# sean-lo/OptimalMatrixCompletion.jl

Hardware: AMD Instinct MI355X
Metric: B&B node-relaxations/sec, 100x100 k=1 (higher is better)
Workload: dtype f64

## Files before the change

optimalmatrixcompletion.jl_amd/csrc/omc_api.cpp:

```cpp
#include <hip/hip_runtime.h>
#include <stdint.h>
#include <limits.h>
#include <stdio.h>
#include <stdlib.h>
#include <string.h>
#include <math.h>
#include <chrono>
#include <string>
#include <vector>
#include <algorithm>
#include <atomic>
#include <thread>
#include <mutex>

#include "omc.h"
#include "omc_device.h"
#include "omc_altmin.h"
#include "omc_shor.h"
#include "omc_shor_relax.h"
#include <unordered_map>
#include <dlfcn.h>
#include <execinfo.h>
#include <signal.h>
#include <unistd.h>
#include <rccl/rccl.h>

#include "omc_host.h"

thread_local std::string g_err;

static void knob_set(Tuning& t, const Knob& kb, const char* value) {
  if (kb.flag) t.*kb.flag = value != nullptr;
  else t.*kb.num = value ? atoi(value) : Tuning{}.*kb.num;
}
static void omc_segv_trace(int sig) {
  void* fr[64];
  const int nf = backtrace(fr, 64);
  const char msg[] = "libomc_hip: fatal signal, native frames:\n";
  (void)!write(2, msg, sizeof(msg) - 1);
  backtrace_symbols_fd(fr, nf, 2);
  signal(sig, SIG_DFL);
  raise(sig);
}
static void tuning_from_env(Tuning& t) {
  for (const Knob& kb : OMC_KNOBS) knob_set(t, kb, getenv(kb.name));
}


extern "C" {

const char* omc_last_error(void) { return g_err.c_str(); }
int omc_version(void) { return OMC_VERSION; }
int omc_device_count(void) {
  int c = 0;
  if (hipGetDeviceCount(&c) != hipSuccess) return 0;
  return c;
}

void omc_relax_params_default(omc_relax_params* p) {
  p->eps_gap = 1e-6; p->eps_feas = 1e-7; p->max_iters = 3000; p->check_every = 25;
  p->rho_scale = 1.0; p->rho_f_ratio = 0.1; p->relax = 1.6; p->time_limit = 3600.0;
  p->reference_quirk_q1 = 1; p->breakpoints = OMC_SMALLEST_1_EIGVEC; p->stall_checks = 8;
  p->bump_max = 2; p->bump_ratio = 4.0; p->bump_factor = 4.0; p->bump_after = 100; p->bump_window = 4; p->slots = 0;
  p->accel = 0; p->aa_mem = 10; p->aa_every = 10; p->aa_start = 50; p->aa_reg = 1e-10; p->aa_safeguard = 1.0; p->first_wins = 0;
  p->early_stop_after = 400; p->early_stop_factor = 1.5;
}

static int upload(DevBuf& b, const void* src, size_t bytes, hipStream_t s) {
  int rc = b.ensure(bytes ? bytes : 8);
  if (rc) return rc;
  if (bytes) HIPCHK(hipMemcpyAsync(b.p, src, bytes, hipMemcpyHostToDevice, s));
  return 0;
}

static int build_colprox_lists(omc_instance* h, int block_min, bool pair_on) {
  if (h->lists_valid && h->lists_block_min == block_min && h->lists_pair == pair_on) return 0;
  const int m = h->m, lds_c = cp_block_lds_cmax(), max_c = cp_block_cmax();
  std::vector<int> solo, wide, blk, slab;
  std::vector<uint8_t> isb(m, 0);
  h->cpb_cl = h->cpb_cs = h->crest_max = h->nrest = 0;
  for (int j0 = 0; j0 < m; j0 += 2) {
    const int j1 = j0 + 1;
    const int c0 = h->col_ptr[j0 + 1] - h->col_ptr[j0], c1 = (j1 < m) ? h->col_ptr[j1 + 1] - h->col_ptr[j1] : 0;
    const bool paired = j1 < m && c0 <= 32 && c1 <= 32;
    for (int j = j0; j <= j1 && j < m; ++j) {
      const int c = (j == j0) ? c0 : c1;
      if (c == 0) continue;
      if (!(paired && pair_on) && c >= block_min && c <= max_c) {
        isb[j] = 1;
        if (c <= lds_c) { blk.push_back(j); h->cpb_cl = std::max(h->cpb_cl, c); } else { slab.push_back(j); h->cpb_cs = std::max(h->cpb_cs, c); }
        continue;
      }
      ++h->nrest; h->crest_max = std::max(h->crest_max, c);
      if (paired) continue;
      if (c <= 64) wide.push_back(j); else solo.push_back(j);
    }
  }
  h->nsolo = (int)solo.size(); h->nwide = (int)wide.size(); h->nblock = (int)blk.size(); h->nslab = (int)slab.size();
  int rc = 0;
  if (h->nsolo && (rc = upload(h->dsolo, solo.data(), sizeof(int) * solo.size(), h->stream))) return rc;
  if (h->nwide && (rc = upload(h->dwide, wide.data(), sizeof(int) * wide.size(), h->stream))) return rc;
  if (h->nblock && (rc = upload(h->dblock, blk.data(), sizeof(int) * blk.size(), h->stream))) return rc;
  if (h->nslab && (rc = upload(h->dslab, slab.data(), sizeof(int) * slab.size(), h->stream))) return rc;
  if ((rc = upload(h->disblock, isb.data(), (size_t)m, h->stream))) return rc;
  HIPCHK(hipStreamSynchronize(h->stream));
  h->lists_valid = true; h->lists_block_min = block_min; h->lists_pair = pair_on;
  return 0;
}

int omc_instance_create(int n, int m, int k, const double* A, const uint8_t* mask, double gamma, int device,
                        omc_instance** out) {
  if (!out) return fail(OMC_ERR_ARGUMENT, "out is NULL");
  *out = nullptr;
  if (!A || !mask) return fail(OMC_ERR_ARGUMENT, "A / mask is NULL");
  if (n <= 0 || m <= 0) return fail(OMC_ERR_DIMENSION, "Dimension mismatch: A must have size (n, m) (OMC.jl:240-246)");
  if (!(n <= m)) return fail(OMC_ERR_DIMENSION, "Input matrix A must have size (n, m) with n <= m (OMC.jl:249-254)");
  if (k < 1 || k > n) return fail(OMC_ERR_ARGUMENT, "rank k must satisfy 1 <= k <= n");
  if (k > 8) return fail(OMC_ERR_UNSUPPORTED, "k > 8 is not supported by this build");
  if (!(gamma > 0.0)) return fail(OMC_ERR_ARGUMENT, "gamma must be positive");
  int ndev = 0;
  if (hipGetDeviceCount(&ndev) != hipSuccess || ndev <= 0)
    return fail(OMC_ERR_NO_DEVICE, "no HIP device visible: the HIP path is the product, there is no CPU fallback");
  if (device < 0 || device >= ndev) return fail(OMC_ERR_ARGUMENT, "device index out of range");
  HIPCHK(hipSetDevice(device));
  omc_instance* h = new omc_instance();
  tuning_from_env(h->tun);
  if (h->tun.segv_trace) { signal(SIGSEGV, omc_segv_trace); signal(SIGABRT, omc_segv_trace); }
  struct Guard { omc_instance*& p; ~Guard() { if (p) omc_instance_destroy(p); } } guard{h};
  h->n = n; h->m = m; h->k = k; h->gamma = gamma; h->device = device;
  { int khz = 0; if (hipDeviceGetAttribute(&khz, hipDeviceAttributeWallClockRate, device) == hipSuccess && khz > 0) h->wall_khz = khz; else (void)hipGetLastError(); }
  h->A.assign(A, A + (size_t)n * m);
  h->mask.resize((size_t)n * m);
  for (size_t e = 0; e < (size_t)n * m; ++e) h->mask[e] = mask[e] ? 1 : 0;
  h->col_ptr.assign(m + 1, 0);
  for (int j = 0; j < m; ++j) {
    int c = 0;
    for (int i = 0; i < n; ++i)
      if (h->mask[(size_t)j * n + i]) { h->col_idx.push_back(i); h->col_val.push_back(A[(size_t)j * n + i]); ++c; }
    h->col_ptr[j + 1] = h->col_ptr[j] + c;
    h->cmax = std::max(h->cmax, c);
  }
  h->nnz = h->col_ptr[m];
  h->sumA2 = 0;
  for (double v : h->col_val) h->sumA2 += v * v;
  h->Ncnt.assign((size_t)n * n, 0.0);
  for (int j = 0; j < m; ++j)
    for (int p = h->col_ptr[j]; p < h->col_ptr[j + 1]; ++p)
      for (int q = h->col_ptr[j]; q < h->col_ptr[j + 1]; ++q)
        h->Ncnt[(size_t)h->col_idx[q] * n + h->col_idx[p]] += 1.0;
  h->row_ptr.assign(n + 1, 0);
  for (int i = 0; i < n; ++i) {
    int c = 0;
    for (int j = 0; j < m; ++j)
      if (h->mask[(size_t)j * n + i]) { h->row_idx.push_back(j); h->row_val.push_back(A[(size_t)j * n + i]); ++c; }
    h->row_ptr[i + 1] = h->row_ptr[i] + c;
  }
  HIPCHK(hipStreamCreate(&h->stream));
  int rc = 0;
  if ((rc = upload(h->drow_ptr, h->row_ptr.data(), sizeof(int) * (n + 1), h->stream))) return rc;
  if ((rc = upload(h->drow_idx, h->row_idx.data(), sizeof(int) * h->nnz_rows(), h->stream))) return rc;
  if ((rc = upload(h->drow_val, h->row_val.data(), sizeof(double) * h->nnz_rows(), h->stream))) return rc;
  if ((rc = upload(h->dA, h->A.data(), sizeof(double) * n * m, h->stream))) return rc;
  if ((rc = upload(h->dmask, h->mask.data(), (size_t)n * m, h->stream))) return rc;
  if ((rc = upload(h->dcol_ptr, h->col_ptr.data(), sizeof(int) * (m + 1), h->stream))) return rc;
  if ((rc = build_colprox_lists(h, h->tun.colprox_block_min, !h->tun.no_colprox_pair))) return rc;
  if ((rc = upload(h->dcol_idx, h->col_idx.data(), sizeof(int) * h->nnz, h->stream))) return rc;
  if ((rc = upload(h->dcol_val, h->col_val.data(), sizeof(double) * h->nnz, h->stream))) return rc;
  if ((rc = upload(h->dNcnt, h->Ncnt.data(), sizeof(double) * n * n, h->stream))) return rc;
  HIPCHK(hipStreamSynchronize(h->stream));
  int lrc = omc_set_max_lds();
  if (lrc) return fail(lrc, "hipFuncSetAttribute(MaxDynamicSharedMemorySize) failed");
  { int arc = omc_altmin_set_lds(); if (arc) return fail(5000 + arc, "hipFuncSetAttribute(MaxDynamicSharedMemorySize) failed for the altmin kernel"); }
  omc_relax_params_default(&h->params);
  *out = h;
  h = nullptr;
  return 0;
}

int omc_instance_create_bits(int n, int m, int k, const double* A, const uint64_t* chunks, double gamma, int device,
                             omc_instance** out) {
  if (!chunks) return fail(OMC_ERR_ARGUMENT, "chunks is NULL");
  if (n <= 0 || m <= 0) return fail(OMC_ERR_DIMENSION, "Dimension mismatch (OMC.jl:240-246)");
  std::vector<uint8_t> mask((size_t)n * m);
  for (size_t e = 0; e < (size_t)n * m; ++e) mask[e] = (uint8_t)((chunks[e >> 6] >> (e & 63)) & 1ull);
  return omc_instance_create(n, m, k, A, mask.data(), gamma, device, out);
}

void omc_instance_destroy(omc_instance* h) {
  if (!h) return;
  if (h->worker.joinable()) h->worker.join();
  (void)hipSetDevice(h->device);
  (void)omc_comm_destroy(h);
  for (hipStream_t q : {h->stream, h->gs[0], h->gs[1], h->gs[2], h->append_stream, h->fetch_stream}) if (q) (void)hipStreamDestroy(q);
  for (int q = 0; q < 2; ++q) for (hipEvent_t e : h->ev_pool[q]) (void)hipEventDestroy(e);
  for (hipEvent_t e : h->ev_up) if (e) (void)hipEventDestroy(e);
  if (h->ev_gram) (void)hipEventDestroy(h->ev_gram);
  for (int q = 0; q < 5; ++q) for (hipEvent_t e : {h->gev[q], h->gevc[q]}) if (e) (void)hipEventDestroy(e);
  if (h->ev_main) (void)hipEventDestroy(h->ev_main);
// ... 225 lines not shown
  w.bump_max = P.bump_max; w.bump_ratio = P.bump_ratio; w.bump_factor = P.bump_factor; w.bump_after = P.bump_after;
  w.bump_gap = P.bump_window * std::max(1, P.check_every);
  w.accel = P.accel ? 1 : 0; w.aa_mem = std::max(2, std::min(P.aa_mem, AA_MAXMEM)); w.aa_every = std::max(1, P.aa_every);
  w.aa_start = std::max(2, P.aa_start); w.aa_reg = P.aa_reg; w.aa_safeguard = P.aa_safeguard;
  {
    std::vector<double> hr((size_t)B + extra_nodes, w.rho);
    if (h->rho_scale_per_node.size() == (size_t)B)
      for (int b = 0; b < B; ++b) hr[b] = w.rho / P.rho_scale * h->rho_scale_per_node[b];
    h->rho_scale_per_node.clear();
    int r0 = upload(h->brhon, hr.data(), sizeof(double) * hr.size(), h->stream); if (r0) return r0;
    HIPCHK(hipStreamSynchronize(h->stream));
    w.rho_node = h->brhon.as<double>();
    r0 = h->brho.ensure(sizeof(double) * (size_t)S); if (r0) return r0;
    w.rho_b = h->brho.as<double>();
  }
  w.relax = P.relax; w.eps_gap = P.eps_gap; w.eps_feas = P.eps_feas;
  w.check_every = std::max(1, P.check_every); w.early_stop_after = P.early_stop_after; w.early_stop_factor = (P.first_wins ? 0.0 : P.early_stop_factor);
  {
    int r0 = h->bgap.ensure(sizeof(double) * 2 * (size_t)S); if (r0) return r0;
    r0 = h->bvotes.ensure(sizeof(int) * (size_t)S); if (r0) return r0;
    r0 = h->bslotlist.ensure(sizeof(int) * (size_t)S); if (r0) return r0;
    w.gap_prev = h->bgap.as<double>(); w.gap_rate = h->bgap.as<double>() + S; w.slow_votes = h->bvotes.as<int>();
    w.slot_list = nullptr;
  }
  std::vector<double> wY((size_t)n * n);
  for (size_t e = 0; e < (size_t)n * n; ++e) wY[e] = shor ? 3.0 : P.rho_f_ratio * h->Ncnt[e] + 2.0;
  int rc_ = 0;
  if ((rc_ = upload(h->dwY, wY.data(), sizeof(double) * n * n, h->stream))) return rc_;
  w.col_ptr = h->dcol_ptr.as<int>(); w.col_idx = h->dcol_idx.as<int>(); w.col_val = h->dcol_val.as<double>();
  const int cp_force = h->cp_force;
  h->cp_force = 0;
  {
    const bool pair_on = !h->tun.no_colprox_pair && cp_force != 2;
    if ((rc_ = build_colprox_lists(h, cp_force == 1 ? INT_MAX : cp_force == 2 ? 1 : h->tun.colprox_block_min, pair_on))) return rc_;
    w.cp_pair = pair_on ? 1 : 0;
  }
  w.cp_nblock = h->nblock; w.cp_block = h->nblock ? h->dblock.as<int>() : nullptr;
  w.cp_nslab = h->nslab; w.cp_slab = h->nslab ? h->dslab.as<int>() : nullptr;
  w.cp_isblock = (h->nblock + h->nslab) ? h->disblock.as<unsigned char>() : nullptr; w.cp_nrest = h->nrest; w.cp_nfact = nullptr;
  w.cone_512 = h->tun.cone_512 ? 1 : 0; w.cp_series = CP_SERIES; w.cp_maxpass = CP_MAXPASS; w.cp_xcd = h->tun.colprox_no_xcd ? 0 : 1;
  w.cp_nsolo = h->nsolo; w.cp_solo = h->nsolo ? h->dsolo.as<int>() : nullptr;
  w.cp_nwide = h->nwide; w.cp_wide = h->nwide ? h->dwide.as<int>() : nullptr;
  w.Ncnt = h->dNcnt.as<double>(); w.wY1 = h->dwY.as<double>();
  w.row_ptr = h->drow_ptr.as<int>(); w.row_idx = h->drow_idx.as<int>();
#define ENS(buf, bytes) do { int r_ = (buf).ensure(bytes); if (r_) return r_; } while (0)
  const size_t sB = (size_t)S;
  const size_t sN = (size_t)B + (size_t)extra_nodes;
  ENS(h->bY, sB * n * n * 8); ENS(h->bYp, sB * n * n * 8); ENS(h->bU, sB * n * k * 8);
  ENS(h->bD1, sB * n * n * 8); ENS(h->bD3, sB * n * n * 8); ENS(h->bW1, sB * n * n * 8); ENS(h->bE3, sB * n * n * 8);
  ENS(h->bdS, sB * rmax * rmax * 8);
  ENS(h->bsm, sB * ((size_t)4 * rmax * k + 3 * k * k) * 8);
  ENS(h->balpha, sB * h->nnz * 8); ENS(h->balphaX, sB * h->nnz * 8); ENS(h->bsval, sB * m * 8);
  ENS(h->bMchk, sB * n * n * 8); ENS(h->bchk, sB * n * k * 8 + (32 + 8 * sB) * 8);
  ENS(h->bG, sB * Rmax * Rmax * 8); ENS(h->blam, sB * Rmax * 8);
  ENS(h->bscal, sB * 16 * 8); ENS(h->bbx, sB * n * 8); ENS(h->bint, sB * 10 * sizeof(int));
  w.np16 = (n + 15) & ~15;
  ENS(h->bMbuf, sB * w.np16 * w.np16 * 8); ENS(h->bVrow, sB * w.np16 * w.np16 * 8);
  ENS(h->blamD, sB * m * n * 8);
  HIPCHK(hipMemsetAsync(h->blamD.p, 0, sB * m * n * 8, h->stream));
  w.lamD = h->blamD.as<double>();
  w.lamDX = nullptr;
  if (n > 144 || shor) {
    ENS(h->blamDX, sB * m * n * 8);
    HIPCHK(hipMemsetAsync(h->blamDX.p, 0, sB * m * n * 8, h->stream));
    w.lamDX = h->blamDX.as<double>();
  }
  w.Mbuf = h->bMbuf.as<double>(); w.Vrow = h->bVrow.as<double>();
  {
    ENS(h->bXs, sB * w.np16 * 16 * 8); ENS(h->bsubS, sB * (17 + 256) * 8); ENS(h->bsubI, sB * 15 * sizeof(int));
    HIPCHK(hipMemsetAsync(h->bXs.p, 0, sB * w.np16 * 16 * 8, h->stream));
    HIPCHK(hipMemsetAsync(h->bsubS.p, 0, sB * (17 + 256) * 8, h->stream));
    HIPCHK(hipMemsetAsync(h->bsubI.p, 0, sB * 15 * sizeof(int), h->stream));
    w.Xs = h->bXs.as<double>(); w.sub_theta = h->bsubS.as<double>(); w.trM = h->bsubS.as<double>() + sB * 16;
    w.sub_on = h->bsubI.as<int>(); w.cone_done = h->bsubI.as<int>() + sB; w.sub_stat = h->bsubI.as<int>() + 2 * sB; w.sub_wait = h->bsubI.as<int>() + 10 * sB; w.sub_nfail = h->bsubI.as<int>() + 11 * sB;
    w.V3 = h->bsubS.as<double>() + sB * 17; w.v3valid = h->bsubI.as<int>() + 12 * sB;
// ... 1839 lines not shown
```

optimalmatrixcompletion.jl_amd/csrc/omc_colprox.hip:

```cpp
#include <hip/hip_runtime.h>
#include <type_traits>
#include <stdint.h>
#include "omc_device.h"
#include "omc_wave.h"

template <int Q>
__device__ __forceinline__ double half_bcast(double v) {
  int lo = __double2loint(v), hi = __double2hiint(v);
  lo = __builtin_amdgcn_update_dpp(0, lo, 0x150 + (Q & 15), 0xF, 0xF, false);
  hi = __builtin_amdgcn_update_dpp(0, hi, 0x150 + (Q & 15), 0xF, 0xF, false);
  auto a = __builtin_amdgcn_permlane16_swap(lo, lo, false, false);
  auto c = __builtin_amdgcn_permlane16_swap(hi, hi, false, false);
  return (Q < 16) ? __hiloint2double(c[0], a[0]) : __hiloint2double(c[1], a[1]);
}
__device__ __forceinline__ double half_sum(double v) {
  v = group_sum_dpp<16>(v);
  const int lo = __double2loint(v), hi = __double2hiint(v);
  auto a = __builtin_amdgcn_permlane16_swap(lo, lo, false, false);
  auto c = __builtin_amdgcn_permlane16_swap(hi, hi, false, false);
  return __hiloint2double(c[0], a[0]) + __hiloint2double(c[1], a[1]);
}
#define CPP_LDS_DOUBLES (64 + 64 + 32)

template <int LPC>
__device__ __forceinline__ double lanes_sum(double v) { if constexpr (LPC == 32) return half_sum(v); else return wave_sum(v); }
#define RQ(q) (((q) < 32) ? R0[(q) & 31] : R1[((NC > 32) ? (q) : 0) & 31])
typedef double dbl2_lds __attribute__((ext_vector_type(2), may_alias));
template <int LPC>
__device__ __forceinline__ void colprox_sweep(const OmcWS& w, const int b, const int lane, const int j, const int off, const int c, const int cmax,
                                              double* st, double* vo_s, int* sidx) {
  constexpr int NC = LPC;
  const int h = (LPC == 32) ? (lane >> 5) : 0, l = lane & (LPC - 1), hb = h * LPC;
  const bool act = l < c;
  const int n = w.n;
  const double gm = w.gamma;
  const double* Y = w.Y + (size_t)b * n * n;
  const double* Yp = w.Yp + (size_t)b * n * n;
  const double* Yx = w.Yx ? w.Yx + (size_t)b * n * n : nullptr;
  double* alpha = w.alpha + (size_t)b * w.nnz + off;
  const double a_reg = act ? w.col_val[off + l] : 0.0;
  const int my = act ? w.col_idx[off + l] : 0;
  const double vo_r = act ? alpha[l] : 0.0;
  sidx[lane] = my; vo_s[lane] = vo_r;
  const double rho_f = w.rho_b[b] * w.rho_f_ratio;
  const double coef = gm / (2.0 * rho_f), cp = gm * gm / (2.0 * rho_f);
  double R0[32], R1[(NC > 32) ? 32 : 1], sc;
  const dbl2_lds* st2 = (const dbl2_lds*)st;
  auto gather = [&](double shift) __attribute__((always_inline)) {
#pragma unroll
    for (int qb = 0; qb < NC; qb += 8) {
      if (qb < cmax) {
        double y1[8], y2[8], vq[8];
#pragma unroll
        for (int u = 0; u < 8; ++u) {
          const int iq = sidx[hb + qb + u];
          vq[u] = vo_s[hb + qb + u];
          const size_t a = (l > qb + u) ? (size_t)iq * n + my : (size_t)my * n + iq;
          y1[u] = Yx ? Yx[a] : Y[a]; y2[u] = Yx ? 0.0 : Yp[a];
// ... 59 lines not shown
    st[lane] = v;
    double a0 = 0.0, a1 = 0.0, a2 = 0.0, a3 = 0.0;
#pragma unroll
    for (int qb = 0; qb < NC; qb += 4) {
      if (qb < cm) {
        if constexpr (LPC == 32) {
          const dbl2_lds s01 = st2[(hb + qb) >> 1], s23 = st2[((hb + qb) >> 1) + 1];
          a0 = fma(RQ(qb), s01.x, a0); a1 = fma(RQ(qb + 1), s01.y, a1);
          a2 = fma(RQ(qb + 2), s23.x, a2); a3 = fma(RQ(qb + 3), s23.y, a3);
        } else {
          a0 = fma(RQ(qb), st[hb + qb], a0); a1 = fma(RQ(qb + 1), st[hb + qb + 1], a1);
          a2 = fma(RQ(qb + 2), st[hb + qb + 2], a2); a3 = fma(RQ(qb + 3), st[hb + qb + 3], a3);
        }
      }
    }
    return -sc * ((a0 + a1) + (a2 + a3));
  };
  const double sprev = (j < w.m) ? w.sval[(size_t)b * w.m + j] : 0.0;
  double s = (sprev > 0.0) ? sprev : 0.0;
  double lo = 0.0, hi = -1.0;
  bool lo_valid = false, fin = (c == 0);
  double yout = 0.0;
  const double ser_lim = (w.cp_series >= 6) ? 5e-3 : 1e-5;
  int npass = 0; double dr_first = -1.0; int why = 0;
  for (int it = 0; it <= 60; ++it) {
    if (!__any(!fin)) break;
    const bool last = (it >= w.cp_maxpass);
    gather(cp * s);
    const bool ok_ = invert();
    if (!fin) ++npass;
    double v[6] = {0.0, 0.0, 0.0, 0.0, 0.0, 0.0};
    double rhs = a_reg, yy = 0.0, yz = 0.0, zz = 0.0;
    bool want_ser = false; double dstep = 0.0;
    int K = 2;
    for (int sv = 0; sv < K; ++sv) {
      const double x = apply(rhs);
      rhs = x;
#pragma unroll
      for (int q = 0; q < 6; ++q) v[q] = (sv == q) ? x : v[q];
      if (sv == 0 && last) { if (!fin) { yout = x; fin = true; } break; }
      if (sv == 1) {
        yy = lanes_sum<LPC>(v[0] * v[0]); yz = lanes_sum<LPC>(v[0] * v[1]); zz = lanes_sum<LPC>(v[1] * v[1]);
        bool big = false;
        if (!fin) {
          if (!ok_) {
            lo = s; lo_valid = false;
            s = (hi > 0.0) ? 0.5 * (s + hi) : (2.0 * s + 1.0);
          } else {
            const double ph = yy - s, dph = -2.0 * cp * yz - 1.0, ddph = 6.0 * cp * cp * zz;
            if (ph >= 0.0) { lo = s; lo_valid = true; } else { hi = s; }
            const double den = 2.0 * dph * dph - ph * ddph;
            double sn = s + ((den > dph * dph) ? (-2.0 * ph * dph / den) : (-ph / dph));
            bool guarded = false;
            if (!(sn > lo) && !lo_valid) { sn = 0.5 * (lo + s); guarded = true; }
            if (sn < lo) { sn = lo; guarded = true; }
            if (hi > 0.0 && sn > hi) { sn = 0.5 * (lo + hi); guarded = true; }
            const double d = sn - s;
            const double dr = (yy > 0.0) ? cp * fabs(d) * sqrt(zz / yy) : 1.0;
            if (dr_first < 0.0) { dr_first = dr; why = guarded ? 1 : 0; }
            if (fabs(d) <= 1e-13 * fmax(1.0, fabs(s))) { fin = true; yout = v[0]; }
            else if (!guarded && dr < ser_lim) { want_ser = true; dstep = d; big = dr >= 1e-5; }
            else s = sn;
          }
        }
        if (__any(want_ser)) K = __any(want_ser && big) ? 6 : 3;
      }
    }
    if (K > 2) {
      double mo[13];
      mo[2] = yy; mo[3] = yz; mo[4] = zz;
#pragma unroll
      for (int i = 2; i < 6; ++i) {
        if (i < K) { mo[2 * i + 1] = lanes_sum<LPC>(v[i - 1] * v[i]); mo[2 * i + 2] = lanes_sum<LPC>(v[i] * v[i]); }
        else { mo[2 * i + 1] = 0.0; mo[2 * i + 2] = 0.0; }
      }
      if (want_ser) {
        double cf[11];
#pragma unroll
        for (int p = 2; p <= 12; ++p) {
          const int cnt = (p <= K + 1) ? p - 1 : ((p <= 2 * K) ? 2 * K - p + 1 : 0);
          cf[p - 2] = (double)cnt * mo[p];
        }
        double d = dstep;
        bool conv = false;
        for (int nt = 0; nt < 8; ++nt) {
          const double t = -cp * d;
          double G = 0.0, dG = 0.0;
#pragma unroll
          for (int q = 10; q >= 0; --q) { dG = fma(dG, t, G); G = fma(G, t, cf[q]); }
          const double F = G - s - d, dF = -cp * dG - 1.0;
          const double dn = d - F / dF;
          conv = fabs(dn - d) <= 1e-14 * fmax(fabs(s), fabs(dn));
          d = dn;
          if (conv) break;
        }
        const double t = cp * d;
        const double t2 = t * t;
        const double lastterm = ((K == 6) ? t2 * t2 * fabs(t) : t2) * sqrt(fmax((K == 6) ? mo[12] : mo[6], 0.0));
        const double growth = sqrt(fmax((K == 6) ? mo[12] : mo[6], 0.0) / fmax((K == 6) ? mo[10] : mo[4], 1e-300));
        if (conv && s + d > lo * (lo_valid ? 1.0 : 0.0) && lastterm * fabs(t) * growth <= 2e-15 * sqrt(yy) && fabs(t) * growth < 0.05) {
          double acc = 0.0;
#pragma unroll
          for (int q = 5; q >= 0; --q) acc = (q < K) ? fma(acc, -t, v[q]) : acc;
          yout = acc; s = s + d; fin = true;
        } else {
          s = s + dstep;
        }
      }
    }
  }
  if (w.sub_debug == 4 && l == 0 && c > 0) {
    atomicAdd(&w.stamps[(npass < 7) ? npass : 7], 1.0);
    if (dr_first >= 0.0) { const int bin = (dr_first > 0.0) ? (int)fmin(15.0, fmax(0.0, -log10(dr_first))) : 15; atomicAdd(&w.stamps[8 + bin], 1.0); if (why) atomicAdd(&w.stamps[24], 1.0); }
    else atomicAdd(&w.stamps[25], 1.0);
  }
  if (act) {
    alpha[l] = yout;
    w.lamD[((size_t)b * w.m + j) * n + my] = yout;
    if (l == 0) w.sval[(size_t)b * w.m + j] = s;
  }
}


#undef RQ
__global__ void __launch_bounds__(256) __attribute__((amdgpu_waves_per_eu(3))) k_colprox_pair(OmcWS w) {
  extern __shared__ double smem[];
  const int wave_in_blk = __builtin_amdgcn_readfirstlane(threadIdx.x >> 6), lane = threadIdx.x & 63, wpb = blockDim.x >> 6;
  const int gw = xcd_block(w.cp_xcd) * wpb + wave_in_blk;
  const int mp = (w.m + 1) >> 1;
  const int bl = gw / mp, pr = gw - bl * mp;
  if (bl >= w.nB) return;
  const int b = slot_of(w, bl);
  if (w.done[b]) return;
  const int j0 = 2 * pr, j1 = j0 + 1;
  const int off0 = w.col_ptr[j0], c0 = w.col_ptr[j0 + 1] - off0;
  const int off1 = (j1 < w.m) ? w.col_ptr[j1] : 0, c1 = (j1 < w.m) ? w.col_ptr[j1 + 1] - off1 : 0;
  if (c0 > 32 || c1 > 32 || j1 >= w.m) return;
  const int cmax = __builtin_amdgcn_readfirstlane((c0 > c1) ? c0 : c1);
  if (cmax == 0) return;
  double* st = smem + (size_t)wave_in_blk * CPP_LDS_DOUBLES;
  double* vo_s = st + 64;
  int* sidx = (int*)(vo_s + 64);
  const int h = lane >> 5;
  colprox_sweep<32>(w, b, lane, j0 + h, h ? off1 : off0, h ? c1 : c0, cmax, st, vo_s, sidx);
}

__global__ void __launch_bounds__(256) __attribute__((amdgpu_waves_per_eu(2))) k_colprox_wide(OmcWS w) {
  extern __shared__ double smem[];
  const int wave_in_blk = __builtin_amdgcn_readfirstlane(threadIdx.x >> 6), lane = threadIdx.x & 63, wpb = blockDim.x >> 6;
  const int gw = xcd_block(w.cp_xcd) * wpb + wave_in_blk;
  const int bl = gw / w.cp_nwide, jj = gw - bl * w.cp_nwide;
  if (bl >= w.nB) return;
  const int b = slot_of(w, bl);
  if (w.done[b]) return;
  const int j = w.cp_wide[jj];
  const int off = w.col_ptr[j], c = w.col_ptr[j + 1] - off;
  const int cmax = __builtin_amdgcn_readfirstlane(c);
  if (cmax == 0 || cmax > 64) return;
  double* st = smem + (size_t)wave_in_blk * CPP_LDS_DOUBLES;
  double* vo_s = st + 64;
  int* sidx = (int*)(vo_s + 64);
  colprox_sweep<64>(w, b, lane, j, off, c, cmax, st, vo_s, sidx);
}


extern "C" void omc_launch_colprox_sweep(const OmcWS* w, hipStream_t s) {
  const int wpb = 4;
  const int wp = w->nB * ((w->m + 1) / 2);
  hipLaunchKernelGGL(k_colprox_pair, dim3((wp + wpb - 1) / wpb), dim3(wpb * 64), (size_t)wpb * CPP_LDS_DOUBLES * sizeof(double), s, *w);
  if (w->cp_nwide > 0) {
    const int ww = w->nB * w->cp_nwide;
    hipLaunchKernelGGL(k_colprox_wide, dim3((ww + wpb - 1) / wpb), dim3(wpb * 64), (size_t)wpb * CPP_LDS_DOUBLES * sizeof(double), s, *w);
  }
}

extern "C" void omc_colprox_sweep_residency(int* pair, int* wide) {
  const int wpb = 4;
  const size_t lds = (size_t)wpb * CPP_LDS_DOUBLES * sizeof(double);
  if (hipOccupancyMaxActiveBlocksPerMultiprocessor(pair, (const void*)k_colprox_pair, wpb * 64, lds) != hipSuccess) *pair = -1;
  if (hipOccupancyMaxActiveBlocksPerMultiprocessor(wide, (const void*)k_colprox_wide, wpb * 64, lds) != hipSuccess) *wide = -1;
}
```

optimalmatrixcompletion.jl_amd/csrc/omc_device.h:

```cpp
#ifndef OMC_DEVICE_H
#define OMC_DEVICE_H
#include <hip/hip_runtime.h>
#include <stdint.h>

#define ROW_TRACE 0
#define ROW_BOX 1
#define ROW_BOUND 2
#define ROW_CUT 3

#define CONE_CLIP01 0
#define CONE_EVALS 2
#define CONE_SEP 3
#define CONE_TOPK 4
#define CONE_BIG 5
#define SMALL_PROJ 0
#define SMALL_RECOVER 1

#define OMC_ST_OPTIMAL 0
#define OMC_ST_SLOW 1
#define OMC_ST_TIME 2
#define OMC_ST_INFEASIBLE 3

#include "omc_layout.h"

// ... 47 lines not shown
  double* trM;
  double* V3; int* v3valid;
  int *sub_wait, *sub_nfail;
  int *sub_on, *cone_done;
  int* ws_first; int ws_phase;
  int* ws_need;
  int sub_guard;
  int* sep_done;
  int cert_enable; double *XsC, *sub_thetaC, *trMc, *lb_est; int *sub_onC, *confirm;
  int shor;
  int shN;
  const double *shP0, *shD0;
  double clip_hi;
  double inv_s2;
  const int *load_from, *save_to;
  double *pY, *pD1, *pD3, *pU, *palpha, *psval, *pXs, *ptheta, *pscal;
  int mw_budget; int* mw_stat; double* ev_out;
  int* sub_stat;
  int* R;
  int *rkind, *rcut, *rbi, *rbj;
  double* rcoef;
  double* rrhs;
  double* cutx;
  double* G;
  int setup_gram_inline;
  double* lam;
  double *obj, *objout, *objprev, *lbprev, *lb, *c0, *evsum, *cpen, *cst, *rp, *rd, *lmin;
  double* bx;
  int *done, *status, *iters, *sweeps, *stall;
  int* rowov;
  OmcGeom geo;
  double* cp_scratch;
  int cp_pair; int cp_nsolo; const int* cp_solo;
  int cp_nwide; const int* cp_wide;
  int cp_nrest;
  int cp_nblock, cp_nslab; const int *cp_block, *cp_slab; const unsigned char* cp_isblock; double* cp_bslab; int* cp_nfact;
  double* Yx;
  int cone_512;
  int cp_series;
  int cp_maxpass;
  int cp_xcd;
  double *cone_scratch, *glob_scratch, *small_scratch;
  double* chk_scratch;
  double* stamps;
  int accel, aa_mem, aa_every, aa_start, aa_dim;
  double aa_reg, aa_safeguard;
  double *aa_F, *aa_G, *aa_zin;
  double* aa_fn;
  int *aa_hist, *aa_head, *aa_pending, *aa_valid, *aa_nacc, *aa_nrej;
};
#define AA_MAXMEM 10

#ifdef __cplusplus
extern "C" {
#endif
void omc_launch_setup(const OmcWS* w, hipStream_t s);
void omc_launch_setup_gram(const OmcWS* w, const int* jobs, int njobs, int nnodes, hipStream_t s);
void omc_launch_colprox(const OmcWS* w, int mode, hipStream_t s);
void omc_launch_cone(const OmcWS* w, int mode, hipStream_t s);
void omc_launch_global(const OmcWS* w, hipStream_t s);
void omc_launch_small(const OmcWS* w, int mode, hipStream_t s);
void omc_launch_cone_ws(const OmcWS* w, hipStream_t s);
void omc_launch_cone_mw(const OmcWS* w, hipStream_t s);
void omc_launch_cone_sub(const OmcWS* w, hipStream_t s);
void omc_launch_check_zero(const OmcWS* w, hipStream_t s);
void omc_launch_check_build(const OmcWS* w, hipStream_t s);
// ... 23 lines not shown
```

optimalmatrixcompletion.jl_amd/csrc/omc_host.h:

```cpp
#pragma once
#include <hip/hip_runtime.h>
#include <stdint.h>
#include <atomic>
#include <mutex>
#include <string>
#include <thread>
#include <unordered_map>
#include <vector>

#include "omc.h"
#include "omc_device.h"
#include "omc_shor_relax.h"

extern thread_local std::string g_err;
static inline int fail(int code, const std::string& msg) { g_err = msg; return code; }
#define HIPCHK(x)                                                                                         \
  do {                                                                                                    \
    hipError_t e_ = (x);                                                                                  \
    if (e_ != hipSuccess) {                                                                               \
      g_err = std::string(#x) + ": " + hipGetErrorString(e_);                                             \
      return (int)e_ > 0 ? (int)e_ : 999;                                                                 \
    }                                                                                                     \
  } while (0)

struct DevBuf {
  void* p = nullptr; size_t cap = 0;
  DevBuf() = default;
  DevBuf(const DevBuf&) = delete;
  DevBuf& operator=(const DevBuf&) = delete;
  ~DevBuf() { release(); }
  int ensure(size_t bytes) {
    if (bytes <= cap) return 0;
    if (p) (void)hipFree(p);
    p = nullptr; cap = 0;
    size_t want = bytes + bytes / 4 + 256;
    hipError_t e = hipMalloc(&p, want);
    if (e != hipSuccess) { g_err = std::string("hipMalloc: ") + hipGetErrorString(e); return (int)e; }
    cap = want;
    return 0;
  }
  void release() { if (p) (void)hipFree(p); p = nullptr; cap = 0; }
  template <class T> T* as() { return (T*)p; }
};
// ... 2 lines not shown
  void* p = nullptr; size_t cap = 0;
  PinBuf() = default;
  PinBuf(const PinBuf&) = delete;
  PinBuf& operator=(const PinBuf&) = delete;
  ~PinBuf() { if (p) (void)hipHostFree(p); }
  int ensure(size_t bytes) {
    if (bytes <= cap) return 0;
    if (p) (void)hipHostFree(p);
    p = nullptr; cap = 0;
    hipError_t e = hipHostMalloc(&p, bytes, hipHostMallocDefault);
    if (e != hipSuccess) { g_err = std::string("hipHostMalloc: ") + hipGetErrorString(e); return (int)e; }
    cap = bytes;
    return 0;
  }
  template <class T> T* as() { return (T*)p; }
};

struct Tuning {
  bool altmin_nolds = false;
  bool colprox_no_xcd = false;
  bool cone_512 = false;
  bool dense_proj = false;
  bool host_phases = false;
  bool global_nolds = false;
  bool no_colprox_pair = false;
  bool no_graph = false;
  bool no_subspace = false;
  bool no_ws_split = false;
  bool segv_trace = false;
  bool setup_gram_inline = false;
  bool shor_explicit = false;
  bool shor_no_subspace = false;
  int check_xs = 16;
  int colprox_block_min = 65;
  int cone_multi_min = 1025;
  int graph_max = 16;
  int harvest_async = 1;
  int harvest_async_min_live = 256;
  int shor_select_kb = 1048576;
  int streams = 4;
  int sub_debug = 0;
  int sub_qmax = 24;
  int timing_stride = 1;
  int ws_quiet = 1;
};
struct Knob { const char* name; bool Tuning::*flag; int Tuning::*num; };
inline const Knob OMC_KNOBS[] = {
  {"OMC_ALTMIN_NOLDS", &Tuning::altmin_nolds, nullptr},      {"OMC_COLPROX_NO_XCD", &Tuning::colprox_no_xcd, nullptr},
  {"OMC_CONE_512", &Tuning::cone_512, nullptr},              {"OMC_DENSE_PROJ", &Tuning::dense_proj, nullptr},
  {"OMC_GLOBAL_NOLDS", &Tuning::global_nolds, nullptr},      {"OMC_HOST_PHASES", &Tuning::host_phases, nullptr},
  {"OMC_NO_COLPROX_PAIR", &Tuning::no_colprox_pair, nullptr},
  {"OMC_NO_GRAPH", &Tuning::no_graph, nullptr},              {"OMC_NO_SUBSPACE", &Tuning::no_subspace, nullptr},
  {"OMC_NO_WS_SPLIT", &Tuning::no_ws_split, nullptr},        {"OMC_SEGV_TRACE", &Tuning::segv_trace, nullptr},
  {"OMC_SETUP_GRAM_INLINE", &Tuning::setup_gram_inline, nullptr},
  {"OMC_SHOR_EXPLICIT", &Tuning::shor_explicit, nullptr},    {"OMC_SHOR_NO_SUBSPACE", &Tuning::shor_no_subspace, nullptr},
  {"OMC_COLPROX_BLOCK_MIN", nullptr, &Tuning::colprox_block_min},
  {"OMC_CHECK_XS", nullptr, &Tuning::check_xs},              {"OMC_CONE_MULTI_MIN", nullptr, &Tuning::cone_multi_min},
  {"OMC_GRAPH_MAX", nullptr, &Tuning::graph_max},            {"OMC_SHOR_SELECT_KB", nullptr, &Tuning::shor_select_kb},
  {"OMC_HARVEST_ASYNC", nullptr, &Tuning::harvest_async},    {"OMC_HARVEST_ASYNC_MIN_LIVE", nullptr, &Tuning::harvest_async_min_live},
  {"OMC_WS_QUIET", nullptr, &Tuning::ws_quiet},
  {"OMC_STREAMS", nullptr, &Tuning::streams},
  {"OMC_SUB_DEBUG", nullptr, &Tuning::sub_debug},            {"OMC_SUB_QMAX", nullptr, &Tuning::sub_qmax},
  {"OMC_TIMING_STRIDE", nullptr, &Tuning::timing_stride},
};

struct omc_instance {
  int n = 0, m = 0, k = 0, device = 0, nnz = 0, cmax = 0;
  double gamma = 0, sumA2 = 0;
  std::vector<int> col_ptr, col_idx; std::vector<double> col_val;
  std::vector<double> A; std::vector<uint8_t> mask;
  std::vector<double> Ncnt;
  std::vector<int> row_ptr, row_idx; std::vector<double> row_val;
  DevBuf drow_ptr, drow_idx, drow_val, aR, arkind, arcut, arbi, arbj, arcoef, arrhs, acutx, aU0, aU, aV, aobj, aint, aG, aG2;
  hipStream_t stream = nullptr;
  Tuning tun;
  hipStream_t gs[3] = {};
  hipEvent_t gev[5] = {};
  hipEvent_t gevc[5] = {};
  hipEvent_t ev_main = nullptr;
  PinBuf pin_flags[2], pin_list[2], pin_done, pin_jobs; DevBuf bgramjobs;
  hipEvent_t ev_up[4] = {}; bool ev_up_rec[4] = {}; hipEvent_t ev_gram = nullptr; bool ev_gram_rec = false;
  double host_ms[OMC_HOST_NPHASE] = {0}; int64_t host_cnt[OMC_HOST_NPHASE] = {0};
  DevBuf dA, dmask, dcol_ptr, dcol_idx, dcol_val, dNcnt, dwY, dsolo, dwide;
  int nwide = 0;
  int nsolo = 0;
  DevBuf dblock, dslab, disblock, bcpb, bnfact;
  int nblock = 0, nslab = 0, nrest = 0, cpb_cl = 0, cpb_cs = 0, crest_max = 0;
  bool lists_valid = false; int lists_block_min = 0; bool lists_pair = true;
  int cp_force = 0;
  DevBuf bYx, bY, bYp, bU, bD1, bD3, bW1, bE3, bQb, brr, bsm, bdS, balpha, balphaX, bsval, bMchk, bsmall, bchk;
  DevBuf bR, brkind, brcut, brbi, brbj, brcoef, brrhs, bcutx, bG, blam;
  DevBuf bobjcol, baaF, baaG, baaZ, baaS, baaI, bMbufC, bVrowC, bchkS, bchkI;
  DevBuf bslotlist, bgap, bvotes, blamDX, bXsC, bsubSC, bsubIC;
  DevBuf bsubz, bscal, bbx, bint, bcp, bcone, bglob, bXout, bThout, bXin, bMbuf, bVrow, bXs, bsubS, bsubI;
  long long sub_tot[8] = {0};
  DevBuf bmwstat, sbigmw, pjM, pjV, pjW, pjS, pjD, pjI;
  long long mw_tot[5] = {0};
  OmcWS ws{};
  omc_relax_params params{};
  bool staged = false;
  double last_solve_seconds = 0; long long total_sweeps = 0; int last_iters_total = 0;
  std::thread worker; std::atomic<int> worker_running{0}, nodes_done{0}; int worker_rc = 0; std::string worker_err;
  int reserve_nodes = 0, reserve_cuts = 0, node_cap = 0, staged_cut_type = 0; std::atomic<int> Btot_live{0}; bool append_closed = true; std::mutex append_mu; hipStream_t append_stream = nullptr;
  std::atomic<int> hold{0};
  std::vector<int> done_q; size_t done_read = 0; std::mutex done_mu; hipStream_t fetch_stream = nullptr;
  void* comm = nullptr; int comm_rank = 0, comm_world = 1; DevBuf bcomm, amobj; int amobj_B = 0;
  int wall_khz = 0;
  std::vector<double> rho_scale_per_node; DevBuf brho, brhon, blamD, bslotint, boY, boU, boal, bobx, boscal, boint;
  int Btot = 0;
  DevBuf sbits, scb, scx, scz, soff, stot, sout, shi, slo, sexist, shist, sohi, solo, scnt;
  bool shor_ready = false; int shor_W = 0; long long shor_pairs = 0;
  double shor_last_ms = 0; long long shor_last_candidates = 0;
  int64_t shor_sel[4] = {0, 0, 0, 0};
  bool shor_req = false, shor_on = false, shor_keep_V = false, shor_via_base = false; std::vector<int> shor_slackrow; DevBuf soV; double shor_rho = 0.05, shor_r4 = 0.0, shor_r5 = 2.0;
  ShWS sh{}; OmcWS wbig{};
  DevBuf sgInts, sgBytes, sgGroups, sgNodeGroup, sAh, sX, sW, sTh, sV1, sV2, sV3, sD0, sP0, sMbufB, sVrowB, sTq, sPq, sNq, sD5x, sD5t, snu5, sP5x,
      scolpart, sminpart, sminpart2, sfroB, svvB, se1, se2, soX, soW, soTh, sbigscr, sXsB, ssubSB, ssubIB;
  long long big_sub_tot[8] = {0};
  struct ShorListKey { int64_t nq = 0, nsoc = 0; uint64_t hlist = 0; std::vector<int64_t> idx, soc; };
  int64_t reserve_shor_nq = 0; int reserve_shor_lists = 0; bool reserve_shor_set = false;
  std::unordered_map<uint64_t, std::vector<int>> sh_byhash; std::vector<ShorListKey> sh_lists;
// ... 30 lines not shown
```

Measured before the change: 2268.

## Pair columns by length for colprox wave pairing via explicit pair list

Replaces the fixed adjacent-column pairing in the column-prox pair kernel with an explicit pair list. By default, columns with at most 32 rows are sorted by length and neighbours are paired, so each wave's two halves have similar row counts and less work is wasted on the shorter half. It also lets more columns be paired than the adjacent rule allowed, and the launch grid is sized to the pair count instead of m/2. In the sweep, a per-half series order Kh replaces the wave-uniform K in the math, and products are computed without FMA contraction so results stay deterministic. The price is an extra indirection load per wave and a different assignment of columns to the block, wide and solo kernels.

```diff
diff --git a/optimalmatrixcompletion.jl_amd/csrc/omc_api.cpp b/optimalmatrixcompletion.jl_amd/csrc/omc_api.cpp
--- a/optimalmatrixcompletion.jl_amd/csrc/omc_api.cpp
+++ b/optimalmatrixcompletion.jl_amd/csrc/omc_api.cpp
@@ -31,7 +31,7 @@
 
 static void knob_set(Tuning& t, const Knob& kb, const char* value) {
   if (kb.flag) t.*kb.flag = value != nullptr;
-  else t.*kb.num = value ? atoi(value) : Tuning{}.*kb.num;
+  else t.*kb.num = value ? (kb.parse ? kb.parse(value) : atoi(value)) : Tuning{}.*kb.num;
 }
 static void omc_segv_trace(int sig) {
   void* fr[64];
@@ -73,38 +73,37 @@
   return 0;
 }
 
-static int build_colprox_lists(omc_instance* h, int block_min, bool pair_on) {
-  if (h->lists_valid && h->lists_block_min == block_min && h->lists_pair == pair_on) return 0;
+static int build_colprox_lists(omc_instance* h, int block_min, bool pair_on, int pairing) {
+  if (h->lists_valid && h->lists_block_min == block_min && h->lists_pair == pair_on && h->lists_pairing == pairing) return 0;
   const int m = h->m, lds_c = cp_block_lds_cmax(), max_c = cp_block_cmax();
-  std::vector<int> solo, wide, blk, slab;
-  std::vector<uint8_t> isb(m, 0);
+  std::vector<int> solo, wide, blk, slab, pairs, len(m);
+  std::vector<uint8_t> isb(m, 0), in_pair(m, 0);
+  for (int j = 0; j < m; ++j) len[j] = h->col_ptr[j + 1] - h->col_ptr[j];
+  if (pair_on) colprox_make_pairs(len, pairing, pairs, in_pair);
   h->cpb_cl = h->cpb_cs = h->crest_max = h->nrest = 0;
-  for (int j0 = 0; j0 < m; j0 += 2) {
-    const int j1 = j0 + 1;
-    const int c0 = h->col_ptr[j0 + 1] - h->col_ptr[j0], c1 = (j1 < m) ? h->col_ptr[j1 + 1] - h->col_ptr[j1] : 0;
-    const bool paired = j1 < m && c0 <= 32 && c1 <= 32;
-    for (int j = j0; j <= j1 && j < m; ++j) {
-      const int c = (j == j0) ? c0 : c1;
-      if (c == 0) continue;
-      if (!(paired && pair_on) && c >= block_min && c <= max_c) {
-        isb[j] = 1;
-        if (c <= lds_c) { blk.push_back(j); h->cpb_cl = std::max(h->cpb_cl, c); } else { slab.push_back(j); h->cpb_cs = std::max(h->cpb_cs, c); }
-        continue;
-      }
-      ++h->nrest; h->crest_max = std::max(h->crest_max, c);
-      if (paired) continue;
-      if (c <= 64) wide.push_back(j); else solo.push_back(j);
+  for (int j = 0; j < m; ++j) {
+    const int c = len[j];
+    if (c == 0) continue;
+    if (!in_pair[j] && c >= block_min && c <= max_c) {
+      isb[j] = 1;
+      if (c <= lds_c) { blk.push_back(j); h->cpb_cl = std::max(h->cpb_cl, c); } else { slab.push_back(j); h->cpb_cs = std::max(h->cpb_cs, c); }
+      continue;
     }
-  }
+    ++h->nrest; h->crest_max = std::max(h->crest_max, c);
+    if (in_pair[j]) continue;
+    if (c <= 64) wide.push_back(j); else solo.push_back(j);
+  }
+  h->npairs = (int)pairs.size() / 2;
   h->nsolo = (int)solo.size(); h->nwide = (int)wide.size(); h->nblock = (int)blk.size(); h->nslab = (int)slab.size();
   int rc = 0;
   if (h->nsolo && (rc = upload(h->dsolo, solo.data(), sizeof(int) * solo.size(), h->stream))) return rc;
   if (h->nwide && (rc = upload(h->dwide, wide.data(), sizeof(int) * wide.size(), h->stream))) return rc;
+  if (h->npairs && (rc = upload(h->dpairs, pairs.data(), sizeof(int) * pairs.size(), h->stream))) return rc;
   if (h->nblock && (rc = upload(h->dblock, blk.data(), sizeof(int) * blk.size(), h->stream))) return rc;
   if (h->nslab && (rc = upload(h->dslab, slab.data(), sizeof(int) * slab.size(), h->stream))) return rc;
   if ((rc = upload(h->disblock, isb.data(), (size_t)m, h->stream))) return rc;
   HIPCHK(hipStreamSynchronize(h->stream));
-  h->lists_valid = true; h->lists_block_min = block_min; h->lists_pair = pair_on;
+  h->lists_valid = true; h->lists_block_min = block_min; h->lists_pair = pair_on; h->lists_pairing = pairing;
   return 0;
 }
 
@@ -163,7 +162,7 @@
   if ((rc = upload(h->dA, h->A.data(), sizeof(double) * n * m, h->stream))) return rc;
   if ((rc = upload(h->dmask, h->mask.data(), (size_t)n * m, h->stream))) return rc;
   if ((rc = upload(h->dcol_ptr, h->col_ptr.data(), sizeof(int) * (m + 1), h->stream))) return rc;
-  if ((rc = build_colprox_lists(h, h->tun.colprox_block_min, !h->tun.no_colprox_pair))) return rc;
+  if ((rc = build_colprox_lists(h, h->tun.colprox_block_min, !h->tun.no_colprox_pair, h->tun.colprox_pairing))) return rc;
   if ((rc = upload(h->dcol_idx, h->col_idx.data(), sizeof(int) * h->nnz, h->stream))) return rc;
   if ((rc = upload(h->dcol_val, h->col_val.data(), sizeof(double) * h->nnz, h->stream))) return rc;
   if ((rc = upload(h->dNcnt, h->Ncnt.data(), sizeof(double) * n * n, h->stream))) return rc;
@@ -455,7 +454,7 @@
   h->cp_force = 0;
   {
     const bool pair_on = !h->tun.no_colprox_pair && cp_force != 2;
-    if ((rc_ = build_colprox_lists(h, cp_force == 1 ? INT_MAX : cp_force == 2 ? 1 : h->tun.colprox_block_min, pair_on))) return rc_;
+    if ((rc_ = build_colprox_lists(h, cp_force == 1 ? INT_MAX : cp_force == 2 ? 1 : h->tun.colprox_block_min, pair_on, h->tun.colprox_pairing))) return rc_;
     w.cp_pair = pair_on ? 1 : 0;
   }
   w.cp_nblock = h->nblock; w.cp_block = h->nblock ? h->dblock.as<int>() : nullptr;
@@ -464,6 +463,7 @@
   w.cone_512 = h->tun.cone_512 ? 1 : 0; w.cp_series = CP_SERIES; w.cp_maxpass = CP_MAXPASS; w.cp_xcd = h->tun.colprox_no_xcd ? 0 : 1;
   w.cp_nsolo = h->nsolo; w.cp_solo = h->nsolo ? h->dsolo.as<int>() : nullptr;
   w.cp_nwide = h->nwide; w.cp_wide = h->nwide ? h->dwide.as<int>() : nullptr;
+  w.cp_npairs = h->npairs; w.cp_pairs = h->npairs ? h->dpairs.as<int>() : nullptr;
   w.Ncnt = h->dNcnt.as<double>(); w.wY1 = h->dwY.as<double>();
   w.row_ptr = h->drow_ptr.as<int>(); w.row_idx = h->drow_idx.as<int>();
 #define ENS(buf, bytes) do { int r_ = (buf).ensure(bytes); if (r_) return r_; } while (0)
diff --git a/optimalmatrixcompletion.jl_amd/csrc/omc_colpairs.h b/optimalmatrixcompletion.jl_amd/csrc/omc_colpairs.h
--- /dev/null
+++ b/optimalmatrixcompletion.jl_amd/csrc/omc_colpairs.h
@@ -0,0 +1,38 @@
+#pragma once
+#include <algorithm>
+#include <stdint.h>
+#include <vector>
+
+enum { COLPAIR_ADJACENT = 0, COLPAIR_LENGTH = 1 };
+static constexpr int COLPAIR_MAX_ROWS = 32;
+
+inline void colprox_make_pairs(const std::vector<int>& len, int mode, std::vector<int>& pairs, std::vector<uint8_t>& in_pair) {
+  const int m = (int)len.size();
+  pairs.clear(); in_pair.assign(m, 0);
+  if (mode == COLPAIR_ADJACENT) {
+    for (int j0 = 0; j0 + 1 < m; j0 += 2) {
+      const int c0 = len[j0], c1 = len[j0 + 1];
+      if (c0 > COLPAIR_MAX_ROWS || c1 > COLPAIR_MAX_ROWS || std::max(c0, c1) <= 0) continue;
+      pairs.push_back(j0); pairs.push_back(j0 + 1);
+      in_pair[j0] = in_pair[j0 + 1] = 1;
+    }
+    return;
+  }
+  std::vector<int> ord;
+  for (int j = 0; j < m; ++j) if (len[j] >= 1 && len[j] <= COLPAIR_MAX_ROWS) ord.push_back(j);
+  std::sort(ord.begin(), ord.end(), [&](int a, int b) { return len[a] != len[b] ? len[a] < len[b] : a < b; });
+  const int np = (int)ord.size() / 2;
+  for (int p = np - 1; p >= 0; --p) {
+    pairs.push_back(ord[2 * p]); pairs.push_back(ord[2 * p + 1]);
+    in_pair[ord[2 * p]] = in_pair[ord[2 * p + 1]] = 1;
+  }
+}
+
+inline long long colprox_pairs_sweep_units(const std::vector<int>& len, const std::vector<int>& pairs) {
+  long long u = 0;
+  for (size_t p = 0; p + 1 < pairs.size(); p += 2) {
+    const long long cm = std::max(len[pairs[p]], len[pairs[p + 1]]);
+    u += cm * ((cm + 3) / 4);
+  }
+  return u;
+}
diff --git a/optimalmatrixcompletion.jl_amd/csrc/omc_colprox.hip b/optimalmatrixcompletion.jl_amd/csrc/omc_colprox.hip
--- a/optimalmatrixcompletion.jl_amd/csrc/omc_colprox.hip
+++ b/optimalmatrixcompletion.jl_amd/csrc/omc_colprox.hip
@@ -24,6 +24,10 @@
 
 template <int LPC>
 __device__ __forceinline__ double lanes_sum(double v) { if constexpr (LPC == 32) return half_sum(v); else return wave_sum(v); }
+__device__ __forceinline__ double prod_rn(double a, double b) {
+#pragma clang fp contract(off)
+  return a * b;
+}
 #define RQ(q) (((q) < 32) ? R0[(q) & 31] : R1[((NC > 32) ? (q) : 0) & 31])
 typedef double dbl2_lds __attribute__((ext_vector_type(2), may_alias));
 template <int LPC>
@@ -149,7 +153,7 @@
     double v[6] = {0.0, 0.0, 0.0, 0.0, 0.0, 0.0};
     double rhs = a_reg, yy = 0.0, yz = 0.0, zz = 0.0;
     bool want_ser = false; double dstep = 0.0;
-    int K = 2;
+    int K = 2, Kh = 2;
     for (int sv = 0; sv < K; ++sv) {
       const double x = apply(rhs);
       rhs = x;
@@ -157,7 +161,7 @@
       for (int q = 0; q < 6; ++q) v[q] = (sv == q) ? x : v[q];
       if (sv == 0 && last) { if (!fin) { yout = x; fin = true; } break; }
       if (sv == 1) {
-        yy = lanes_sum<LPC>(v[0] * v[0]); yz = lanes_sum<LPC>(v[0] * v[1]); zz = lanes_sum<LPC>(v[1] * v[1]);
+        yy = lanes_sum<LPC>(prod_rn(v[0], v[0])); yz = lanes_sum<LPC>(prod_rn(v[0], v[1])); zz = lanes_sum<LPC>(prod_rn(v[1], v[1]));
         bool big = false;
         if (!fin) {
           if (!ok_) {
@@ -180,6 +184,7 @@
             else s = sn;
           }
         }
+        Kh = want_ser ? (big ? 6 : 3) : 2;
         if (__any(want_ser)) K = __any(want_ser && big) ? 6 : 3;
       }
     }
@@ -188,14 +193,17 @@
       mo[2] = yy; mo[3] = yz; mo[4] = zz;
 #pragma unroll
       for (int i = 2; i < 6; ++i) {
-        if (i < K) { mo[2 * i + 1] = lanes_sum<LPC>(v[i - 1] * v[i]); mo[2 * i + 2] = lanes_sum<LPC>(v[i] * v[i]); }
+        if (i < K) {
+          const double mo_odd = lanes_sum<LPC>(prod_rn(v[i - 1], v[i])), mo_even = lanes_sum<LPC>(prod_rn(v[i], v[i]));
+          mo[2 * i + 1] = (i < Kh) ? mo_odd : 0.0; mo[2 * i + 2] = (i < Kh) ? mo_even : 0.0;
+        }
         else { mo[2 * i + 1] = 0.0; mo[2 * i + 2] = 0.0; }
       }
       if (want_ser) {
         double cf[11];
 #pragma unroll
         for (int p = 2; p <= 12; ++p) {
-          const int cnt = (p <= K + 1) ? p - 1 : ((p <= 2 * K) ? 2 * K - p + 1 : 0);
+          const int cnt = (p <= Kh + 1) ? p - 1 : ((p <= 2 * Kh) ? 2 * Kh - p + 1 : 0);
           cf[p - 2] = (double)cnt * mo[p];
         }
         double d = dstep;
@@ -213,12 +221,12 @@
         }
         const double t = cp * d;
         const double t2 = t * t;
-        const double lastterm = ((K == 6) ? t2 * t2 * fabs(t) : t2) * sqrt(fmax((K == 6) ? mo[12] : mo[6], 0.0));
-        const double growth = sqrt(fmax((K == 6) ? mo[12] : mo[6], 0.0) / fmax((K == 6) ? mo[10] : mo[4], 1e-300));
+        const double lastterm = ((Kh == 6) ? t2 * t2 * fabs(t) : t2) * sqrt(fmax((Kh == 6) ? mo[12] : mo[6], 0.0));
+        const double growth = sqrt(fmax((Kh == 6) ? mo[12] : mo[6], 0.0) / fmax((Kh == 6) ? mo[10] : mo[4], 1e-300));
         if (conv && s + d > lo * (lo_valid ? 1.0 : 0.0) && lastterm * fabs(t) * growth <= 2e-15 * sqrt(yy) && fabs(t) * growth < 0.05) {
           double acc = 0.0;
 #pragma unroll
-          for (int q = 5; q >= 0; --q) acc = (q < K) ? fma(acc, -t, v[q]) : acc;
+          for (int q = 5; q >= 0; --q) acc = (q < Kh) ? fma(acc, -t, v[q]) : acc;
           yout = acc; s = s + d; fin = true;
         } else {
           s = s + dstep;
@@ -244,22 +252,21 @@
   extern __shared__ double smem[];
   const int wave_in_blk = __builtin_amdgcn_readfirstlane(threadIdx.x >> 6), lane = threadIdx.x & 63, wpb = blockDim.x >> 6;
   const int gw = xcd_block(w.cp_xcd) * wpb + wave_in_blk;
-  const int mp = (w.m + 1) >> 1;
-  const int bl = gw / mp, pr = gw - bl * mp;
+  const int np = w.cp_npairs;
+  const int bl = gw / np, pr = gw - bl * np;
   if (bl >= w.nB) return;
   const int b = slot_of(w, bl);
   if (w.done[b]) return;
-  const int j0 = 2 * pr, j1 = j0 + 1;
+  const int j0 = w.cp_pairs[2 * pr], j1 = w.cp_pairs[2 * pr + 1];
   const int off0 = w.col_ptr[j0], c0 = w.col_ptr[j0 + 1] - off0;
-  const int off1 = (j1 < w.m) ? w.col_ptr[j1] : 0, c1 = (j1 < w.m) ? w.col_ptr[j1 + 1] - off1 : 0;
-  if (c0 > 32 || c1 > 32 || j1 >= w.m) return;
+  const int off1 = w.col_ptr[j1], c1 = w.col_ptr[j1 + 1] - off1;
   const int cmax = __builtin_amdgcn_readfirstlane((c0 > c1) ? c0 : c1);
   if (cmax == 0) return;
   double* st = smem + (size_t)wave_in_blk * CPP_LDS_DOUBLES;
   double* vo_s = st + 64;
   int* sidx = (int*)(vo_s + 64);
   const int h = lane >> 5;
-  colprox_sweep<32>(w, b, lane, j0 + h, h ? off1 : off0, h ? c1 : c0, cmax, st, vo_s, sidx);
+  colprox_sweep<32>(w, b, lane, h ? j1 : j0, h ? off1 : off0, h ? c1 : c0, cmax, st, vo_s, sidx);
 }
 
 __global__ void __launch_bounds__(256) __attribute__((amdgpu_waves_per_eu(2))) k_colprox_wide(OmcWS w) {
@@ -283,8 +290,8 @@
 
 extern "C" void omc_launch_colprox_sweep(const OmcWS* w, hipStream_t s) {
   const int wpb = 4;
-  const int wp = w->nB * ((w->m + 1) / 2);
-  hipLaunchKernelGGL(k_colprox_pair, dim3((wp + wpb - 1) / wpb), dim3(wpb * 64), (size_t)wpb * CPP_LDS_DOUBLES * sizeof(double), s, *w);
+  const int wp = w->nB * w->cp_npairs;
+  if (wp > 0) hipLaunchKernelGGL(k_colprox_pair, dim3((wp + wpb - 1) / wpb), dim3(wpb * 64), (size_t)wpb * CPP_LDS_DOUBLES * sizeof(double), s, *w);
   if (w->cp_nwide > 0) {
     const int ww = w->nB * w->cp_nwide;
     hipLaunchKernelGGL(k_colprox_wide, dim3((ww + wpb - 1) / wpb), dim3(wpb * 64), (size_t)wpb * CPP_LDS_DOUBLES * sizeof(double), s, *w);
diff --git a/optimalmatrixcompletion.jl_amd/csrc/omc_device.h b/optimalmatrixcompletion.jl_amd/csrc/omc_device.h
--- a/optimalmatrixcompletion.jl_amd/csrc/omc_device.h
+++ b/optimalmatrixcompletion.jl_amd/csrc/omc_device.h
@@ -103,6 +103,7 @@
   OmcGeom geo;
   double* cp_scratch;
   int cp_pair; int cp_nsolo; const int* cp_solo;
+  int cp_npairs; const int* cp_pairs;
   int cp_nwide; const int* cp_wide;
   int cp_nrest;
   int cp_nblock, cp_nslab; const int *cp_block, *cp_slab; const unsigned char* cp_isblock; double* cp_bslab; int* cp_nfact;
diff --git a/optimalmatrixcompletion.jl_amd/csrc/omc_host.h b/optimalmatrixcompletion.jl_amd/csrc/omc_host.h
--- a/optimalmatrixcompletion.jl_amd/csrc/omc_host.h
+++ b/optimalmatrixcompletion.jl_amd/csrc/omc_host.h
@@ -1,6 +1,7 @@
 #pragma once
 #include <hip/hip_runtime.h>
 #include <stdint.h>
+#include <string.h>
 #include <atomic>
 #include <mutex>
 #include <string>
@@ -9,6 +10,7 @@
 #include <vector>
 
 #include "omc.h"
+#include "omc_colpairs.h"
 #include "omc_device.h"
 #include "omc_shor_relax.h"
 
@@ -77,6 +79,7 @@
   bool shor_explicit = false;
   bool shor_no_subspace = false;
   int check_xs = 16;
+  int colprox_pairing = COLPAIR_LENGTH;
   int colprox_block_min = 65;
   int cone_multi_min = 1025;
   int graph_max = 16;
@@ -89,7 +92,8 @@
   int timing_stride = 1;
   int ws_quiet = 1;
 };
-struct Knob { const char* name; bool Tuning::*flag; int Tuning::*num; };
+struct Knob { const char* name; bool Tuning::*flag; int Tuning::*num; int (*parse)(const char*) = nullptr; };
+inline int colprox_pairing_parse(const char* v) { return (!strcmp(v, "adjacent") || !strcmp(v, "0")) ? COLPAIR_ADJACENT : COLPAIR_LENGTH; }
 inline const Knob OMC_KNOBS[] = {
   {"OMC_ALTMIN_NOLDS", &Tuning::altmin_nolds, nullptr},      {"OMC_COLPROX_NO_XCD", &Tuning::colprox_no_xcd, nullptr},
   {"OMC_CONE_512", &Tuning::cone_512, nullptr},              {"OMC_DENSE_PROJ", &Tuning::dense_proj, nullptr},
@@ -100,6 +104,7 @@
   {"OMC_SETUP_GRAM_INLINE", &Tuning::setup_gram_inline, nullptr},
   {"OMC_SHOR_EXPLICIT", &Tuning::shor_explicit, nullptr},    {"OMC_SHOR_NO_SUBSPACE", &Tuning::shor_no_subspace, nullptr},
   {"OMC_COLPROX_BLOCK_MIN", nullptr, &Tuning::colprox_block_min},
+  {"OMC_COLPROX_PAIRING", nullptr, &Tuning::colprox_pairing, colprox_pairing_parse},
   {"OMC_CHECK_XS", nullptr, &Tuning::check_xs},              {"OMC_CONE_MULTI_MIN", nullptr, &Tuning::cone_multi_min},
   {"OMC_GRAPH_MAX", nullptr, &Tuning::graph_max},            {"OMC_SHOR_SELECT_KB", nullptr, &Tuning::shor_select_kb},
   {"OMC_HARVEST_ASYNC", nullptr, &Tuning::harvest_async},    {"OMC_HARVEST_ASYNC_MIN_LIVE", nullptr, &Tuning::harvest_async_min_live},
@@ -126,12 +131,13 @@
   PinBuf pin_flags[2], pin_list[2], pin_done, pin_jobs; DevBuf bgramjobs;
   hipEvent_t ev_up[4] = {}; bool ev_up_rec[4] = {}; hipEvent_t ev_gram = nullptr; bool ev_gram_rec = false;
   double host_ms[OMC_HOST_NPHASE] = {0}; int64_t host_cnt[OMC_HOST_NPHASE] = {0};
-  DevBuf dA, dmask, dcol_ptr, dcol_idx, dcol_val, dNcnt, dwY, dsolo, dwide;
+  DevBuf dA, dmask, dcol_ptr, dcol_idx, dcol_val, dNcnt, dwY, dsolo, dwide, dpairs;
+  int npairs = 0;
   int nwide = 0;
   int nsolo = 0;
   DevBuf dblock, dslab, disblock, bcpb, bnfact;
   int nblock = 0, nslab = 0, nrest = 0, cpb_cl = 0, cpb_cs = 0, crest_max = 0;
-  bool lists_valid = false; int lists_block_min = 0; bool lists_pair = true;
+  bool lists_valid = false; int lists_block_min = 0; bool lists_pair = true; int lists_pairing = COLPAIR_LENGTH;
   int cp_force = 0;
   DevBuf bYx, bY, bYp, bU, bD1, bD3, bW1, bE3, bQb, brr, bsm, bdS, balpha, balphaX, bsval, bMchk, bsmall, bchk;
   DevBuf bR, brkind, brcut, brbi, brbj, brcoef, brrhs, bcutx, bG, blam;
```

New measurement: 2319 (median of 4 runs). 1.02x the previous value.
